# Dustin-Ray/capyCRYPT

Measured on NVIDIA B200. Metric: sha3_256_GBps, higher is better.
Workload: dtype u64

## Files before the change

### capycrypt_b200/csrc/keccak_bs.cuh

```cuda
#pragma once
#include <cstdint>

#include "keccak.cuh"

namespace capy {

static __device__ const uint2 KECCAK_RC_BITS[32] = {
    {0x50F4F1u, 0x0DB916u}, {0x000000u, 0x8C7F94u}, {0x000000u, 0x000000u}, {0x000000u, 0x327356u},
    {0x000000u, 0x000000u}, {0x000000u, 0x000000u}, {0x000000u, 0x000000u}, {0x000000u, 0xB5D4DEu},
    {0x000000u, 0x000000u}, {0x000000u, 0x000000u}, {0x000000u, 0x000000u}, {0x000000u, 0x000000u},
    {0x000000u, 0x000000u}, {0x000000u, 0x000000u}, {0x000000u, 0x000000u}, {0x000000u, 0xD81C68u},
    {0x000000u, 0x000000u}, {0x000000u, 0x000000u}, {0x000000u, 0x000000u}, {0x000000u, 0x000000u},
    {0x000000u, 0x000000u}, {0x000000u, 0x000000u}, {0x000000u, 0x000000u}, {0x000000u, 0x000000u},
    {0x000000u, 0x000000u}, {0x000000u, 0x000000u}, {0x000000u, 0x000000u}, {0x000000u, 0x000000u},
    {0x000000u, 0x000000u}, {0x000000u, 0x000000u}, {0x000000u, 0x000000u}, {0x000000u, 0xBBE0CCu}};

template <int K>
__device__ __forceinline__ uint32_t bs_from(uint32_t v, uint32_t lane) {
  if constexpr (K % 32 == 0) return v;
  else return __shfl_sync(0xffffffffu, v, (int)(lane - (uint32_t)K));
}

template <int R>
__device__ __forceinline__ void bs_rot(uint32_t (&b)[2], uint32_t t0, uint32_t t1, uint32_t lane) {
  if constexpr (R % 2 == 0) {
    b[0] = bs_from<R / 2>(t0, lane);
    b[1] = bs_from<R / 2>(t1, lane);
  } else {
    b[0] = bs_from<(R + 1) / 2>(t1, lane);
    b[1] = bs_from<(R - 1) / 2>(t0, lane);
  }
}

#define CAPY_BS_RHO_PI(X, Y, R)                                                                       \
  bs_rot<(R)>(b[(Y) + 5 * ((2 * (X) + 3 * (Y)) % 5)],                                                 \
              lop_xor3(a[(X) + 5 * (Y)][0], c[((X) + 4) % 5][0], n[((X) + 1) % 5][0]),                \
              lop_xor3(a[(X) + 5 * (Y)][1], c[((X) + 4) % 5][1], n[((X) + 1) % 5][1]), lane);

__device__ __forceinline__ uint32_t bs_flip_if(uint32_t v, uint32_t rounds, uint32_t round) {
  asm("{\n\t.reg .pred p;\n\t.reg .b32 t;\n\tand.b32 t, %1, %2;\n\tsetp.ne.u32 p, t, 0;\n\t@p not.b32 %0, %0;\n\t}"
      : "+r"(v)
      : "r"(rounds), "r"(round));
  return v;
}

__device__ __forceinline__ void keccak_bs_round(uint32_t (&a)[25][2], uint32_t lane, uint2 rc, uint32_t round) {
  uint32_t c[5][2], n[5][2], b[25][2];
#pragma unroll
  for (int x = 0; x < 5; x++) {
#pragma unroll
    for (int h = 0; h < 2; h++) c[x][h] = lop_xor3(lop_xor3(a[x][h], a[x + 5][h], a[x + 10][h]), a[x + 15][h], a[x + 20][h]);
    n[x][0] = bs_from<1>(c[x][1], lane);
    n[x][1] = c[x][0];
  }
  CAPY_BS_RHO_PI(0, 0, 0)  CAPY_BS_RHO_PI(1, 0, 1)  CAPY_BS_RHO_PI(2, 0, 62) CAPY_BS_RHO_PI(3, 0, 28) CAPY_BS_RHO_PI(4, 0, 27)
  CAPY_BS_RHO_PI(0, 1, 36) CAPY_BS_RHO_PI(1, 1, 44) CAPY_BS_RHO_PI(2, 1, 6)  CAPY_BS_RHO_PI(3, 1, 55) CAPY_BS_RHO_PI(4, 1, 20)
  CAPY_BS_RHO_PI(0, 2, 3)  CAPY_BS_RHO_PI(1, 2, 10) CAPY_BS_RHO_PI(2, 2, 43) CAPY_BS_RHO_PI(3, 2, 25) CAPY_BS_RHO_PI(4, 2, 39)
  CAPY_BS_RHO_PI(0, 3, 41) CAPY_BS_RHO_PI(1, 3, 45) CAPY_BS_RHO_PI(2, 3, 15) CAPY_BS_RHO_PI(3, 3, 21) CAPY_BS_RHO_PI(4, 3, 8)
  CAPY_BS_RHO_PI(0, 4, 18) CAPY_BS_RHO_PI(1, 4, 2)  CAPY_BS_RHO_PI(2, 4, 61) CAPY_BS_RHO_PI(3, 4, 56) CAPY_BS_RHO_PI(4, 4, 14)
#pragma unroll
  for (int y = 0; y < 5; y++) {
#pragma unroll
    for (int x = 0; x < 5; x++) {
#pragma unroll
      for (int h = 0; h < 2; h++)
        a[x + 5 * y][h] = lop_chi(b[x + 5 * y][h], b[(x + 1) % 5 + 5 * y][h], b[(x + 2) % 5 + 5 * y][h]);
    }
  }
  a[0][0] = bs_flip_if(a[0][0], rc.x, round);
  a[0][1] = bs_flip_if(a[0][1], rc.y, round);
}
#undef CAPY_BS_RHO_PI

struct BsTranspose {
  uint32_t rot[5], keep[5];
  __device__ __forceinline__ explicit BsTranspose(uint32_t lane) {
#pragma unroll
    for (int k = 0; k < 5; k++) {
      const uint32_t d = 16u >> k;
      const uint32_t lo_bits = k == 0 ? 0x0000FFFFu : k == 1 ? 0x00FF00FFu : k == 2 ? 0x0F0F0F0Fu : k == 3 ? 0x33333333u : 0x55555555u;
      const bool upper = lane & d;
      rot[k] = upper ? 32u - d : d;
      keep[k] = upper ? ~lo_bits : lo_bits;
    }
  }
  __device__ __forceinline__ uint32_t operator()(uint32_t x) const {
#pragma unroll
    for (int k = 0; k < 5; k++) {
      const uint32_t y = __shfl_xor_sync(0xffffffffu, x, 16u >> k);
      const uint32_t r = __funnelshift_l(y, y, rot[k]);
      asm("lop3.b32 %0, %0, %1, %2, 0xE4;" : "+r"(x) : "r"(r), "r"(keep[k]));
    }
    return x;
  }
};

__device__ __forceinline__ void bs_gather(uint32_t (&w)[2], uint32_t lo, uint32_t hi, uint32_t lane) {
#pragma unroll
  for (int h = 0; h < 2; h++) {
    const int src = (int)(2 * lane + h);
    const uint32_t l = __shfl_sync(0xffffffffu, lo, src);
    const uint32_t u = __shfl_sync(0xffffffffu, hi, src);
    w[h] = lane < 16 ? l : u;
  }
}

__device__ __forceinline__ void bs_scatter(uint32_t& lo, uint32_t& hi, const uint32_t (&w)[2], uint32_t lane) {
  const int src = (int)(lane >> 1);
  const uint32_t l0 = __shfl_sync(0xffffffffu, w[0], src), l1 = __shfl_sync(0xffffffffu, w[1], src);
  const uint32_t u0 = __shfl_sync(0xffffffffu, w[0], src + 16), u1 = __shfl_sync(0xffffffffu, w[1], src + 16);
  lo = lane & 1 ? l1 : l0;
  hi = lane & 1 ? u1 : u0;
}

}
```

### capycrypt_b200/csrc/sha3_api.cu

```cuda
#include <algorithm>
#include <cmath>
#include <cstdlib>
#include <memory>
#include <thread>
#include <type_traits>
#include <vector>

#include "internal.h"
#include "hostbatch.h"
#include "keccak_bs.cuh"
#include "sponge.cuh"

namespace capy {

template <int LANES>
__global__ void __launch_bounds__(128)
    sha3_uniform_kernel(const uint8_t* __restrict__ data, uint64_t stride, uint64_t len, uint32_t suffix,
                        uint8_t* __restrict__ out, uint32_t out_bytes, uint64_t n) {
  const uint64_t i = (uint64_t)blockIdx.x * blockDim.x + threadIdx.x;
  if (i >= n) return;
  constexpr uint64_t RATE = 8ull * LANES;
  const uint2* q = reinterpret_cast<const uint2*>(data + i * stride);
  Lane a[25];
  state_zero(a);
  const uint64_t nfull = len / RATE;
  for (uint64_t b = 0; b < nfull; b++) {
#pragma unroll
    for (int j = 0; j < LANES; j++) {
      uint2 v = __ldg(q + j);
      a[j].lo ^= v.x;
      a[j].hi ^= v.y;
    }
    q += LANES;
    keccak_f1600(a);
  }
  const uint32_t rem = (uint32_t)(len - nfull * RATE);
#pragma unroll
  for (int j = 0; j < LANES; j++) {
    const uint32_t o = 8u * j;
    uint32_t lo = 0, hi = 0;
    if (o < rem) {
      uint2 v = __ldg(q + j);
      lo = v.x;
      hi = v.y;
      if (o + 8 > rem) {
        const uint32_t keep = rem - o;
        if (keep < 4) {
          lo &= (1u << (8 * keep)) - 1u;
          hi = 0;
        } else if (keep > 4) {
          hi &= (1u << (8 * (keep - 4))) - 1u;
        } else {
          hi = 0;
        }
      }
    }
    if (rem >= o && rem < o + 8) {
      const uint32_t k = rem - o;
      if (k < 4) lo |= suffix << (8 * k);
      else hi |= suffix << (8 * (k - 4));
    }
    a[j].lo ^= lo;
    a[j].hi ^= hi;
  }
  if (rem + 1 < RATE) a[LANES - 1].hi ^= 0x80000000u;
  keccak_f1600(a);

  uint8_t* o = out + i * (uint64_t)out_bytes;
  if ((out_bytes & 15u) == 0 && (reinterpret_cast<uintptr_t>(out) & 15u) == 0) {
#pragma unroll
    for (int j = 0; j < 4; j++)
      if (16u * j < out_bytes)
        reinterpret_cast<uint4*>(o)[j] = make_uint4(a[2 * j].lo, a[2 * j].hi, a[2 * j + 1].lo, a[2 * j + 1].hi);
  } else {
#pragma unroll
    for (int j = 0; j < 8; j++) {
      if (8u * j < out_bytes) reinterpret_cast<uint32_t*>(o)[2 * j] = a[j].lo;
      if (8u * j + 4 < out_bytes) reinterpret_cast<uint32_t*>(o)[2 * j + 1] = a[j].hi;
    }
  }
}

template <int LANES, int MSG_LANES>
__global__ void __launch_bounds__(128, 4)
    sha3_short_kernel(const uint4* __restrict__ data, uint64_t stride16, uint32_t suffix, uint4* __restrict__ out,
                      uint32_t out_bytes, uint64_t n) {
  static_assert(MSG_LANES % 2 == 0 && MSG_LANES < LANES, "whole 16-byte loads, one block");
  constexpr int OUT_LANES = (200 - 8 * LANES) / 16;
  const uint32_t lane = threadIdx.x & 31u;
  const uint64_t i = (uint64_t)blockIdx.x * blockDim.x + threadIdx.x;
  if (i - lane >= n) return;
  const bool live = i < n;
  const BsTranspose transpose(lane);

  uint32_t a[25][2];
  {
    const uint4* q = data + i * stride16;
    uint32_t w[2 * MSG_LANES];
#pragma unroll
    for (int j = 0; j < MSG_LANES / 2; j++) {
      const uint4 v = live ? __ldg(q + j) : make_uint4(0u, 0u, 0u, 0u);
      w[4 * j] = v.x;
      w[4 * j + 1] = v.y;
      w[4 * j + 2] = v.z;
      w[4 * j + 3] = v.w;
    }
#pragma unroll
    for (int j = 0; j < 2 * MSG_LANES; j++) w[j] = transpose(w[j]);
#pragma unroll
    for (int l = 0; l < MSG_LANES; l++) bs_gather(a[l], w[2 * l], w[2 * l + 1], lane);
  }
#pragma unroll
  for (int l = MSG_LANES; l < 25; l++) a[l][0] = a[l][1] = 0u;
  const uint32_t pad = (uint32_t)((uint64_t)suffix >> (2 * lane));
  a[MSG_LANES][0] = 0u - (pad & 1u);
  a[MSG_LANES][1] = 0u - ((pad >> 1) & 1u);
  a[LANES - 1][1] ^= lane == 31 ? 0xFFFFFFFFu : 0u;

  const uint2 rc = __ldg(&KECCAK_RC_BITS[lane]);
  keccak_bs_round(a, lane, rc, 1u);
#pragma unroll 1
  for (int r = 1; r < 23; r += 2) {
    keccak_bs_round(a, lane, rc, 1u << r);
    keccak_bs_round(a, lane, rc, 2u << r);
  }
  keccak_bs_round(a, lane, rc, 1u << 23);

  uint32_t w[2 * OUT_LANES];
#pragma unroll
  for (int l = 0; l < OUT_LANES; l++) bs_scatter(w[2 * l], w[2 * l + 1], a[l], lane);
#pragma unroll
  for (int j = 0; j < 2 * OUT_LANES; j++) w[j] = transpose(w[j]);
  if (!live) return;
  uint4* o = out + i * (uint64_t)(out_bytes / 16);
#pragma unroll
  for (int j = 0; j < OUT_LANES / 2; j++) o[j] = make_uint4(w[4 * j], w[4 * j + 1], w[4 * j + 2], w[4 * j + 3]);
}

template <int LANES>
__global__ void prefix_state_kernel(const uint8_t* prefix, uint32_t nblocks, uint64_t* state) {
  if (threadIdx.x != 0 || blockIdx.x != 0) return;
  Lane a[25];
  state_zero(a);
  for (uint32_t b = 0; b < nblocks; b++) {
    const uint8_t* p = prefix + (size_t)b * 8 * LANES;
#pragma unroll
    for (int j = 0; j < LANES; j++) {
      uint64_t v = 0;
      for (int k = 0; k < 8; k++) v |= (uint64_t)p[8 * j + k] << (8 * k);
      a[j].lo ^= (uint32_t)v;
      a[j].hi ^= (uint32_t)(v >> 32);
    }
    keccak_f1600(a);
  }
  for (int k = 0; k < 25; k++) state[k] = ((uint64_t)a[k].hi << 32) | a[k].lo;
}

constexpr uint32_t kLenBins = 1u << 14;
constexpr uint64_t kHostPlanMaxItems = 1ull << 18;

__device__ __forceinline__ uint32_t len_bin(const uint64_t* off, uint64_t i, uint32_t stride_bytes) {
  const uint64_t blocks = (off[i + 1] - off[i]) / stride_bytes;
  return blocks < kLenBins - 1 ? (uint32_t)blocks : kLenBins - 1;
}

__global__ void len_hist_kernel(const uint64_t* __restrict__ off, uint64_t n, uint32_t stride_bytes, uint32_t* hist) {
  const uint64_t i = (uint64_t)blockIdx.x * blockDim.x + threadIdx.x;
  if (i < n) atomicAdd(&hist[len_bin(off, i, stride_bytes)], 1u);
}

__global__ void __launch_bounds__(1024) len_scan_kernel(uint32_t* hist, uint32_t* summary) {
  __shared__ unsigned long long tot_s;
  __shared__ uint32_t max_s, bins_s;
  const uint32_t t = threadIdx.x;
  constexpr uint32_t PER = kLenBins / 1024;
  static_assert(PER == 16, "four uint4 per thread");
  if (t == 0) { tot_s = 0; max_s = 0; bins_s = 0; }
  __syncthreads();
  const uint32_t lo = kLenBins - (t + 1) * PER;
  uint32_t c[PER];
#pragma unroll
  for (int q = 0; q < 4; q++) {
    const uint4 v = reinterpret_cast<const uint4*>(hist + lo)[q];
    c[4 * q] = v.x; c[4 * q + 1] = v.y; c[4 * q + 2] = v.z; c[4 * q + 3] = v.w;
  }
  uint32_t sum = 0, nb = 0, mx = 0;
  unsigned long long tot = 0;
#pragma unroll
  for (int k = 0; k < (int)PER; k++) {
    sum += c[k];
    if (c[k]) { nb++; mx = lo + k; }
    tot += (unsigned long long)c[k] * (lo + k + 1);
  }
  if (sum) {
    atomicAdd(&tot_s, tot);
    atomicMax(&max_s, mx);
    atomicAdd(&bins_s, nb);
  }
  __syncthreads();
  uint32_t incl = sum;
#pragma unroll
  for (int d = 1; d < 32; d <<= 1) {
    const uint32_t v = __shfl_up_sync(0xffffffffu, incl, d);
    if ((t & 31) >= (uint32_t)d) incl += v;
  }
  __shared__ uint32_t wsum[32];
  if ((t & 31) == 31) wsum[t >> 5] = incl;
  __syncthreads();
  if (t < 32) {
    uint32_t w = wsum[t];
#pragma unroll
    for (int d = 1; d < 32; d <<= 1) {
      const uint32_t v = __shfl_up_sync(0xffffffffu, w, d);
      if (t >= (uint32_t)d) w += v;
    }
    wsum[t] = w;
  }
  __syncthreads();
  uint32_t run = incl - sum + ((t >> 5) ? wsum[(t >> 5) - 1] : 0u);
#pragma unroll
  for (int k = (int)PER - 1; k >= 0; k--) {
    const uint32_t cnt = c[k];
    c[k] = run;
    run += cnt;
  }
#pragma unroll
  for (int q = 0; q < 4; q++) reinterpret_cast<uint4*>(hist + lo)[q] = make_uint4(c[4 * q], c[4 * q + 1], c[4 * q + 2], c[4 * q + 3]);
  if (t == 0) {
    summary[0] = (uint32_t)tot_s;
    summary[1] = (uint32_t)(tot_s >> 32);
    summary[2] = max_s;
    summary[3] = bins_s;
  }
}

__global__ void len_scatter_kernel(const uint64_t* __restrict__ off, uint64_t n, uint32_t stride_bytes, uint32_t* cursor,
                                   uint32_t* __restrict__ order) {
  const uint64_t i = (uint64_t)blockIdx.x * blockDim.x + threadIdx.x;
  if (i < n) order[atomicAdd(&cursor[len_bin(off, i, stride_bytes)], 1u)] = (uint32_t)i;
}

constexpr double kPairChainRatio = 3.08 / 4.6;
constexpr int kMaxWarpCosched = 3;
constexpr double kWarpChainRatio[kMaxWarpCosched + 1] = {0.0, 2.06 / 4.6, 2.36 / 4.6, 3.00 / 4.6};

static void plan_tiers(const std::vector<uint32_t>& cum, uint64_t n, uint32_t max_blocks, double total_blocks, int sm_count,
                       uint64_t warp_items[kMaxWarpCosched], uint64_t* pair_items, int force_c = 0) {
  for (int c = 0; c < kMaxWarpCosched; c++) warp_items[c] = 0;
  *pair_items = 0;
  const size_t nb = cum.size();
  std::vector<double> work_above(nb);
  double acc = 0;
  for (size_t k = nb; k-- > 0;) {
    work_above[k] = acc;
    const uint64_t cnt = (k == 0 ? n : cum[k - 1]) - cum[k];
    acc += (double)cnt * (double)(k + 1);
  }
  auto longer_than = [&](double thr, uint64_t* count, double* work) {
    if (thr < 1.0) {
      *count = n;
      *work = total_blocks;
      return;
    }
    const size_t k = std::min<size_t>((size_t)thr - 1, nb - 1);
    *count = cum[k];
    *work = work_above[k];
  };
  const double l1 = (double)max_blocks;
  const int c_first = force_c >= 1 && force_c <= kMaxWarpCosched ? force_c : 1;
  for (double T = l1 * kWarpChainRatio[c_first]; T < l1; T *= 1.01) {
    uint64_t k_above[kMaxWarpCosched + 2];
    double w_above[kMaxWarpCosched + 2];
    k_above[0] = 0;
    w_above[0] = 0;
    for (int c = 1; c <= kMaxWarpCosched; c++) {
      const int next = c + 1;
      const double ratio = next <= kMaxWarpCosched ? kWarpChainRatio[next] : kPairChainRatio;
      longer_than(T / ratio, &k_above[c], &w_above[c]);
      if (force_c && c != force_c) {
        k_above[c] = c < force_c ? 0 : k_above[force_c];
        w_above[c] = c < force_c ? 0 : w_above[force_c];
      }
    }
    uint64_t k_fast;
    double w_fast;
    longer_than(T, &k_fast, &w_fast);
    if (k_above[kMaxWarpCosched] == 0 && T < l1 * kPairChainRatio) continue;
    uint64_t blocks = 0;
    double sm_time = 0;
    uint64_t cnt[kMaxWarpCosched];
    for (int c = 1; c <= kMaxWarpCosched; c++) {
      cnt[c - 1] = k_above[c] - k_above[c - 1];
      blocks += (cnt[c - 1] + 4 * c - 1) / (4 * c);
      sm_time += (w_above[c] - w_above[c - 1]) * kWarpChainRatio[c] / (4.0 * c);
    }
    const uint64_t k_p = k_fast - k_above[kMaxWarpCosched];
    blocks += (k_p + 63) / 64;
    sm_time += (w_fast - w_above[kMaxWarpCosched]) * kPairChainRatio / 64.0 + (total_blocks - w_fast) / 128.0;
    if (blocks + 1 > (uint64_t)sm_count) continue;
    if (sm_time > 0.95 * T * (double)sm_count) continue;
    if ((total_blocks - w_fast) / 128.0 > T * (double)((uint64_t)sm_count - blocks)) continue;
    for (int c = 0; c < kMaxWarpCosched; c++) warp_items[c] = cnt[c];
    *pair_items = k_p;
    return;
  }
}

template <int... Ls, class F>
static int with_lanes(int lanes, F&& f) {
  int rc = CAPY_ERR_BAD_ARG;
  (void)((lanes == Ls && ((rc = f(std::integral_constant<int, Ls>())), true)) || ...);
  return rc;
}

struct CudaFree {
  void operator()(void* p) const { cudaFree(p); }
};
template <class T>
using DevPtr = std::unique_ptr<T, CudaFree>;
template <class T>
static cudaError_t dev_alloc(DevPtr<T>& p, size_t bytes) {
  T* q = nullptr;
  const cudaError_t e = cudaMalloc(&q, bytes);
  if (e == cudaSuccess) p.reset(q);
  return e;
}

struct LenHist {
  uint64_t total_blocks = 0;
  uint32_t max_bin = 0;
  uint32_t bins = 0;
  std::vector<uint32_t> cnt;
};

static void host_len_hist(const uint64_t* h_off, uint64_t n, uint32_t stride_bytes, LenHist* h) {
  h->cnt.assign(kLenBins, 0);
  const double inv = 1.0 / (double)stride_bytes;
  for (uint64_t i = 0; i < n; i++) {
    const uint64_t len = h_off[i + 1] - h_off[i];
    uint64_t q = (uint64_t)((double)len * inv);
    if (q * stride_bytes > len) q--;
    else if ((q + 1) * stride_bytes <= len) q++;
    const uint32_t b = q < kLenBins - 1 ? (uint32_t)q : kLenBins - 1;
    if (h->cnt[b]++ == 0) h->bins++;
    if (b > h->max_bin) h->max_bin = b;
    h->total_blocks += (uint64_t)b + 1;
  }
}

static int device_len_hist(capy_ctx* ctx, cudaStream_t st, const uint64_t* d_off, uint64_t n, uint32_t stride_bytes,
                           uint32_t* hist, LenHist* h) {
  uint32_t* summary = hist + kLenBins;
  CAPY_CUDA(ctx, cudaMemsetAsync(hist, 0, (size_t)kLenBins * 4 + 64, st));
  len_hist_kernel<<<(unsigned)((n + 255) / 256), 256, 0, st>>>(d_off, n, stride_bytes, hist);
  len_scan_kernel<<<1, 1024, 0, st>>>(hist, summary);
  ctx->launches += 2;
  if (!h->cnt.empty()) return CAPY_OK;
  uint32_t h_sum[4];
  CAPY_CUDA(ctx, cudaMemcpyAsync(h_sum, summary, sizeof h_sum, cudaMemcpyDeviceToHost, st));
  CAPY_CUDA(ctx, cudaStreamSynchronize(st));
  h->total_blocks = (uint64_t)h_sum[0] | ((uint64_t)h_sum[1] << 32);
  h->max_bin = h_sum[2];
  h->bins = h_sum[3];
  return CAPY_OK;
}

static int plan_from_hist(capy_ctx* ctx, DeviceCtx& dc, cudaStream_t st, const uint64_t* d_off, uint64_t n,
                          uint32_t stride_bytes, const LenHist& h, uint32_t* hist, uint32_t* order, bool allow_pair,
                          int force_c, LaunchPlan* plan) {
  const uint32_t max_blocks = h.max_bin + 1;
  const double ideal = (double)h.total_blocks / (32.0 * 4.0 * dc.sm_count);
  if (allow_pair && max_blocks > 64 && (double)max_blocks > 1.05 * ideal) {
    std::vector<uint32_t> cum(kLenBins);
    if (!h.cnt.empty()) {
      uint32_t above = 0;
      for (uint32_t k = kLenBins; k-- > 0;) {
        cum[k] = above;
        above += h.cnt[k];
      }
    } else {
      CAPY_CUDA(ctx, cudaMemcpyAsync(cum.data(), hist, (size_t)kLenBins * 4, cudaMemcpyDeviceToHost, st));
      CAPY_CUDA(ctx, cudaStreamSynchronize(st));
    }
    plan_tiers(cum, n, max_blocks, (double)h.total_blocks, dc.sm_count, plan->warp_items, &plan->pair_items, force_c);
  }
  if (h.bins == 1) plan->uniform_blocks = max_blocks;
  if (h.bins > 1) {
    len_scatter_kernel<<<(unsigned)((n + 255) / 256), 256, 0, st>>>(d_off, n, stride_bytes, hist, order);
    ctx->launches++;
    CAPY_CUDA(ctx, cudaGetLastError());
    plan->order = order;
    plan->warps_per_smsp = 0;
    if ((double)max_blocks * 4.0 > 0.7 * ideal) {
      plan->warps_per_smsp = 3;
      if ((double)max_blocks * 3.0 > 0.7 * ideal) plan->warps_per_smsp = 2;
      if ((double)max_blocks * 2.0 > 0.7 * ideal) plan->warps_per_smsp = 1;
    }
  }
  return CAPY_OK;
}

static int plan_ragged(capy_ctx* ctx, DeviceCtx& dc, cudaStream_t st, const uint64_t* d_off, uint64_t n,
                       uint32_t stride_bytes, LaunchPlan* plan, bool allow_pair = true, int force_c = 0) {
  *plan = LaunchPlan();
  if (n < 1 || n > 0xffffffffull) return CAPY_OK;
  const uint64_t* h_off = host_off_find(dc, d_off, n);
  LenHist h;
  if (h_off) {
    const uint64_t len0 = h_off[1] - h_off[0];
    bool uniform = true;
    for (uint64_t i = 1; i < n && uniform; i++) uniform = (h_off[i + 1] - h_off[i]) == len0;
    if (uniform) {
      plan->uniform_blocks = len0 / stride_bytes + 1;
      return CAPY_OK;
    }
    if (n > kHostPlanMaxItems) h_off = nullptr;
    else host_len_hist(h_off, n, stride_bytes, &h);
  }
  const bool cached = ctx->plan_cache.load() != 0 && force_c == 0 && !h_off;
  if (cached) {
    for (PlanEntry& e : dc.plans)
      if (e.off == d_off && e.n == n && e.unit == stride_bytes && e.allow_pair == allow_pair) {
        e.last_use = ++dc.use_clock;
        *plan = e.plan;
        return CAPY_OK;
      }
  }
  uint32_t* hist = (uint32_t*)scratch_get(dc, st, kPlanHist, (size_t)kLenBins * 4 + 64);
  DevPtr<uint32_t> owned;
  if (cached && dev_alloc(owned, (size_t)n * 4) != cudaSuccess) {
    cudaGetLastError();
    return CAPY_ERR_OOM;
  }
  uint32_t* order = cached ? owned.get() : (uint32_t*)scratch_get(dc, st, kPlanOrder, (size_t)n * 4);
  if (!hist || !order) return CAPY_ERR_OOM;
// ... 1210 lines not shown
```

Measured before the change: 310.5.

## Permute bitsliced lane order to drop gather/scatter shuffles and pair-wise transposes

```diff
diff --git a/capycrypt_b200/csrc/keccak_bs.cuh b/capycrypt_b200/csrc/keccak_bs.cuh
--- a/capycrypt_b200/csrc/keccak_bs.cuh
+++ b/capycrypt_b200/csrc/keccak_bs.cuh
@@ -15,42 +15,54 @@
     {0x000000u, 0x000000u}, {0x000000u, 0x000000u}, {0x000000u, 0x000000u}, {0x000000u, 0x000000u},
     {0x000000u, 0x000000u}, {0x000000u, 0x000000u}, {0x000000u, 0x000000u}, {0x000000u, 0xBBE0CCu}};
 
+static __constant__ uint32_t BS_POW2[32] = {
+    1u << 0,  1u << 1,  1u << 2,  1u << 3,  1u << 4,  1u << 5,  1u << 6,  1u << 7,  1u << 8,  1u << 9,  1u << 10,
+    1u << 11, 1u << 12, 1u << 13, 1u << 14, 1u << 15, 1u << 16, 1u << 17, 1u << 18, 1u << 19, 1u << 20, 1u << 21,
+    1u << 22, 1u << 23, 1u << 24, 1u << 25, 1u << 26, 1u << 27, 1u << 28, 1u << 29, 1u << 30, 1u << 31};
+
+__device__ __forceinline__ uint32_t bs_sigma(uint32_t lane) { return (lane >> 1) | ((lane & 1u) << 4); }
+
 template <int K>
-__device__ __forceinline__ uint32_t bs_from(uint32_t v, uint32_t lane) {
+__device__ __forceinline__ uint32_t bs_src(uint32_t sigma) {
+  return __umulhi(sigma * BS_POW2[27] + ((32u - K) << 27), 66u);
+}
+
+template <int K>
+__device__ __forceinline__ uint32_t bs_from(uint32_t v, uint32_t sigma) {
   if constexpr (K % 32 == 0) return v;
-  else return __shfl_sync(0xffffffffu, v, (int)(lane - (uint32_t)K));
+  else return __shfl_sync(0xffffffffu, v, (int)bs_src<K>(sigma));
 }
 
 template <int R>
-__device__ __forceinline__ void bs_rot(uint32_t (&b)[2], uint32_t t0, uint32_t t1, uint32_t lane) {
+__device__ __forceinline__ void bs_rot(uint32_t (&b)[2], uint32_t t0, uint32_t t1, uint32_t sigma) {
   if constexpr (R % 2 == 0) {
-    b[0] = bs_from<R / 2>(t0, lane);
-    b[1] = bs_from<R / 2>(t1, lane);
+    b[0] = bs_from<R / 2>(t0, sigma);
+    b[1] = bs_from<R / 2>(t1, sigma);
   } else {
-    b[0] = bs_from<(R + 1) / 2>(t1, lane);
-    b[1] = bs_from<(R - 1) / 2>(t0, lane);
+    b[0] = bs_from<(R + 1) / 2>(t1, sigma);
+    b[1] = bs_from<(R - 1) / 2>(t0, sigma);
   }
 }
 
 #define CAPY_BS_RHO_PI(X, Y, R)                                                                       \
   bs_rot<(R)>(b[(Y) + 5 * ((2 * (X) + 3 * (Y)) % 5)],                                                 \
               lop_xor3(a[(X) + 5 * (Y)][0], c[((X) + 4) % 5][0], n[((X) + 1) % 5][0]),                \
-              lop_xor3(a[(X) + 5 * (Y)][1], c[((X) + 4) % 5][1], n[((X) + 1) % 5][1]), lane);
+              lop_xor3(a[(X) + 5 * (Y)][1], c[((X) + 4) % 5][1], n[((X) + 1) % 5][1]), sigma);
 
-__device__ __forceinline__ uint32_t bs_flip_if(uint32_t v, uint32_t rounds, uint32_t round) {
-  asm("{\n\t.reg .pred p;\n\t.reg .b32 t;\n\tand.b32 t, %1, %2;\n\tsetp.ne.u32 p, t, 0;\n\t@p not.b32 %0, %0;\n\t}"
-      : "+r"(v)
-      : "r"(rounds), "r"(round));
-  return v;
+__device__ __forceinline__ uint32_t bs_iota(uint32_t v, uint32_t& q) {
+  const uint32_t two = BS_POW2[1];
+  const uint32_t k = (uint32_t)__mulhi((int)q, (int)two);
+  q *= two;
+  return v * (k * two + 1u) + k;
 }
 
-__device__ __forceinline__ void keccak_bs_round(uint32_t (&a)[25][2], uint32_t lane, uint2 rc, uint32_t round) {
+__device__ __forceinline__ void keccak_bs_round(uint32_t (&a)[25][2], uint32_t sigma, uint32_t (&q)[2]) {
   uint32_t c[5][2], n[5][2], b[25][2];
 #pragma unroll
   for (int x = 0; x < 5; x++) {
 #pragma unroll
     for (int h = 0; h < 2; h++) c[x][h] = lop_xor3(lop_xor3(a[x][h], a[x + 5][h], a[x + 10][h]), a[x + 15][h], a[x + 20][h]);
-    n[x][0] = bs_from<1>(c[x][1], lane);
+    n[x][0] = bs_from<1>(c[x][1], sigma);
     n[x][1] = c[x][0];
   }
   CAPY_BS_RHO_PI(0, 0, 0)  CAPY_BS_RHO_PI(1, 0, 1)  CAPY_BS_RHO_PI(2, 0, 62) CAPY_BS_RHO_PI(3, 0, 28) CAPY_BS_RHO_PI(4, 0, 27)
@@ -67,50 +79,57 @@
         a[x + 5 * y][h] = lop_chi(b[x + 5 * y][h], b[(x + 1) % 5 + 5 * y][h], b[(x + 2) % 5 + 5 * y][h]);
     }
   }
-  a[0][0] = bs_flip_if(a[0][0], rc.x, round);
-  a[0][1] = bs_flip_if(a[0][1], rc.y, round);
+  a[0][0] = bs_iota(a[0][0], q[0]);
+  a[0][1] = bs_iota(a[0][1], q[1]);
 }
 #undef CAPY_BS_RHO_PI
 
+__device__ __forceinline__ uint32_t lop_mux(uint32_t a, uint32_t b, uint32_t m) {
+  uint32_t d;
+  asm("lop3.b32 %0, %1, %2, %3, 0xE4;" : "=r"(d) : "r"(a), "r"(b), "r"(m));
+  return d;
+}
+
+__device__ __forceinline__ void bs_interleave(uint32_t& lo, uint32_t& hi) {
+  const uint32_t l = lo, h = hi;
+  lo = lop_mux(l, h * BS_POW2[1], 0x55555555u);
+  hi = lop_mux(__umulhi(l, BS_POW2[31]), h, 0x55555555u);
+}
+
 struct BsTranspose {
-  uint32_t rot[5], keep[5];
+  uint32_t sel_send[2], sel_x1[2], sel_x2[2], mul_send[3], mul_recv[3], keep[3];
   __device__ __forceinline__ explicit BsTranspose(uint32_t lane) {
+    sel_send[0] = lane & 16u ? 0x5410u : 0x3276u;
+    sel_x1[0] = lane & 16u ? 0x3276u : 0x5410u;
+    sel_x2[0] = lane & 16u ? 0x3254u : 0x7610u;
+    sel_send[1] = lane & 8u ? 0x6240u : 0x3715u;
+    sel_x1[1] = lane & 8u ? 0x3715u : 0x6240u;
+    sel_x2[1] = lane & 8u ? 0x3614u : 0x7250u;
 #pragma unroll
-    for (int k = 0; k < 5; k++) {
-      const uint32_t d = 16u >> k;
-      const uint32_t lo_bits = k == 0 ? 0x0000FFFFu : k == 1 ? 0x00FF00FFu : k == 2 ? 0x0F0F0F0Fu : k == 3 ? 0x33333333u : 0x55555555u;
+    for (int k = 0; k < 3; k++) {
+      const uint32_t d = 4u >> k;
+      const uint32_t lo_bits = k == 0 ? 0x0F0F0F0Fu : k == 1 ? 0x33333333u : 0x55555555u;
       const bool upper = lane & d;
-      rot[k] = upper ? 32u - d : d;
+      mul_send[k] = upper ? BS_POW2[d] : BS_POW2[32 - d];
+      mul_recv[k] = upper ? BS_POW2[32 - d] : BS_POW2[d];
       keep[k] = upper ? ~lo_bits : lo_bits;
     }
   }
-  __device__ __forceinline__ uint32_t operator()(uint32_t x) const {
+  __device__ __forceinline__ void operator()(uint32_t& x1, uint32_t& x2) const {
 #pragma unroll
-    for (int k = 0; k < 5; k++) {
-      const uint32_t y = __shfl_xor_sync(0xffffffffu, x, 16u >> k);
-      const uint32_t r = __funnelshift_l(y, y, rot[k]);
-      asm("lop3.b32 %0, %0, %1, %2, 0xE4;" : "+r"(x) : "r"(r), "r"(keep[k]));
+    for (int k = 0; k < 2; k++) {
+      const uint32_t y = __shfl_xor_sync(0xffffffffu, __byte_perm(x1, x2, sel_send[k]), 16u >> k);
+      x1 = __byte_perm(x1, y, sel_x1[k]);
+      x2 = __byte_perm(x2, y, sel_x2[k]);
     }
-    return x;
+#pragma unroll
+    for (int k = 0; k < 3; k++) {
+      const uint32_t s = lop_mux(x2 * mul_send[k] + __umulhi(x2, mul_send[k]), x1, keep[k]);
+      const uint32_t y = __shfl_xor_sync(0xffffffffu, s, 4u >> k);
+      x1 = lop_mux(x1, y * mul_recv[k] + __umulhi(y, mul_recv[k]), keep[k]);
+      x2 = lop_mux(x2, y, keep[k]);
+    }
   }
 };
 
-__device__ __forceinline__ void bs_gather(uint32_t (&w)[2], uint32_t lo, uint32_t hi, uint32_t lane) {
-#pragma unroll
-  for (int h = 0; h < 2; h++) {
-    const int src = (int)(2 * lane + h);
-    const uint32_t l = __shfl_sync(0xffffffffu, lo, src);
-    const uint32_t u = __shfl_sync(0xffffffffu, hi, src);
-    w[h] = lane < 16 ? l : u;
-  }
 }
-
-__device__ __forceinline__ void bs_scatter(uint32_t& lo, uint32_t& hi, const uint32_t (&w)[2], uint32_t lane) {
-  const int src = (int)(lane >> 1);
-  const uint32_t l0 = __shfl_sync(0xffffffffu, w[0], src), l1 = __shfl_sync(0xffffffffu, w[1], src);
-  const uint32_t u0 = __shfl_sync(0xffffffffu, w[0], src + 16), u1 = __shfl_sync(0xffffffffu, w[1], src + 16);
-  lo = lane & 1 ? l1 : l0;
-  hi = lane & 1 ? u1 : u0;
-}
-
-}
diff --git a/capycrypt_b200/csrc/sha3_api.cu b/capycrypt_b200/csrc/sha3_api.cu
--- a/capycrypt_b200/csrc/sha3_api.cu
+++ b/capycrypt_b200/csrc/sha3_api.cu
@@ -92,6 +92,7 @@
   if (i - lane >= n) return;
   const bool live = i < n;
   const BsTranspose transpose(lane);
+  const uint32_t sigma = bs_sigma(lane);
 
   uint32_t a[25][2];
   {
@@ -106,31 +107,38 @@
       w[4 * j + 3] = v.w;
     }
 #pragma unroll
-    for (int j = 0; j < 2 * MSG_LANES; j++) w[j] = transpose(w[j]);
-#pragma unroll
-    for (int l = 0; l < MSG_LANES; l++) bs_gather(a[l], w[2 * l], w[2 * l + 1], lane);
+    for (int l = 0; l < MSG_LANES; l++) {
+      bs_interleave(w[2 * l], w[2 * l + 1]);
+      transpose(w[2 * l], w[2 * l + 1]);
+      a[l][0] = w[2 * l];
+      a[l][1] = w[2 * l + 1];
+    }
   }
 #pragma unroll
   for (int l = MSG_LANES; l < 25; l++) a[l][0] = a[l][1] = 0u;
-  const uint32_t pad = (uint32_t)((uint64_t)suffix >> (2 * lane));
+  const uint32_t pad = (uint32_t)((uint64_t)suffix >> (2 * sigma));
   a[MSG_LANES][0] = 0u - (pad & 1u);
   a[MSG_LANES][1] = 0u - ((pad >> 1) & 1u);
-  a[LANES - 1][1] ^= lane == 31 ? 0xFFFFFFFFu : 0u;
-
-  const uint2 rc = __ldg(&KECCAK_RC_BITS[lane]);
-  keccak_bs_round(a, lane, rc, 1u);
+  a[LANES - 1][1] ^= sigma == 31 ? 0xFFFFFFFFu : 0u;
+
+  const uint2 rc = __ldg(&KECCAK_RC_BITS[sigma]);
+  uint32_t q[2] = {__brev(rc.x), __brev(rc.y)};
+  keccak_bs_round(a, sigma, q);
 #pragma unroll 1
   for (int r = 1; r < 23; r += 2) {
-    keccak_bs_round(a, lane, rc, 1u << r);
-    keccak_bs_round(a, lane, rc, 2u << r);
-  }
-  keccak_bs_round(a, lane, rc, 1u << 23);
+    keccak_bs_round(a, sigma, q);
+    keccak_bs_round(a, sigma, q);
+  }
+  keccak_bs_round(a, sigma, q);
 
   uint32_t w[2 * OUT_LANES];
 #pragma unroll
-  for (int l = 0; l < OUT_LANES; l++) bs_scatter(w[2 * l], w[2 * l + 1], a[l], lane);
-#pragma unroll
-  for (int j = 0; j < 2 * OUT_LANES; j++) w[j] = transpose(w[j]);
+  for (int l = 0; l < OUT_LANES; l++) {
+    w[2 * l] = a[l][0];
+    w[2 * l + 1] = a[l][1];
+    transpose(w[2 * l], w[2 * l + 1]);
+    bs_interleave(w[2 * l], w[2 * l + 1]);
+  }
   if (!live) return;
   uint4* o = out + i * (uint64_t)(out_bytes / 16);
 #pragma unroll
```

New measurement: 306.6 (median of 6 runs). 0.988x the previous value.
